# Unalome81/IEEE-802.11-OFDM-QPSK-Simulator

Hardware: AMD Instinct MI355X
Metric: OFDM symbols/sec (whole node) over BER-vs-SNR sweep; achieved HBM GB/s vs peak (higher is better)
Workload: dtype f32

## Files before the change

### ieee-802.11-ofdm-qpsk-simulator_amd/csrc/ofdm_capi.hip

```cpp
#include <hip/hip_runtime.h>
#include <algorithm>
#include <cmath>
#include <cstdint>
#include <cstdlib>
#include <complex>
#include <cstdio>
#include <cstring>
#include <mutex>
#include <string>
#include <vector>
#include "ofdm_internal.h"
#include "ofdm_ctx.h"

using namespace ofdm;

namespace ofdm {

thread_local std::string g_last_error;

int set_error(int code, const char *fmt, ...) {
    char buf[512];
    va_list ap;
    va_start(ap, fmt);
    vsnprintf(buf, sizeof(buf), fmt, ap);
// ... 171 lines not shown
        return set_error(OFDM_E_HIP, "hipStreamCreate failed");
    }
    c->stream = c->own;
    for (int conv = 0; conv < 2; ++conv) {
        std::vector<float2> t;
        host_ltf_time(conv, t);
        std::vector<float2> t2(68 * 2);
        for (int r = 0; r < 68; ++r) {
            const float2 v = t[(r - 4 + 64) & 63];
            t2[2 * r] = t2[2 * r + 1] = make_float2(2.0f * v.x, 2.0f * v.y);
        }
        if (hipMalloc(&c->d_ltf[conv], 64 * sizeof(float2)) != hipSuccess ||
            hipMemcpy(c->d_ltf[conv], t.data(), 64 * sizeof(float2), hipMemcpyHostToDevice) != hipSuccess ||
            hipMalloc(&c->d_ltf2_rows[conv], t2.size() * sizeof(float2)) != hipSuccess ||
            hipMemcpy(c->d_ltf2_rows[conv], t2.data(), t2.size() * sizeof(float2), hipMemcpyHostToDevice) != hipSuccess) {
            ofdm_ctx_destroy(reinterpret_cast<ofdm_ctx *>(c));
            return set_error(OFDM_E_NOMEM, "LTF table upload failed");
        }
    }
    *out = reinterpret_cast<ofdm_ctx *>(c);
    return OFDM_OK;
}

int ofdm_ctx_destroy(ofdm_ctx *ctx) {
    Ctx *c = reinterpret_cast<Ctx *>(ctx);
    if (!c) return OFDM_OK;
    hipSetDevice(c->device);
    hipStreamSynchronize(c->stream);
    for (auto &e : c->done) { hipEventDestroy(e.a); hipEventDestroy(e.b); }
    for (auto &e : c->open) { hipEventDestroy(e.a); hipEventDestroy(e.b); }
    for (auto ev : c->pool) hipEventDestroy(ev);
    if (c->tx_stream) hipStreamSynchronize(c->tx_stream);
    for (void *p : {(void *)c->d_ltf[0], (void *)c->d_ltf[1], (void *)c->d_ltf2_rows[0], (void *)c->d_ltf2_rows[1], c->d_tx, c->d_bits, c->d_cnt, c->d_scratch,
                    c->d_scratch2, c->d_wave, c->d_tx2, c->d_bits2, c->d_work})
        if (p) hipFree(p);
    for (hipEvent_t ev : {c->ev_start, c->ev_tx[0], c->ev_tx[1], c->ev_rx[0], c->ev_rx[1]})
        if (ev) hipEventDestroy(ev);
    if (c->h_cnt) hipHostFree(c->h_cnt);
    if (c->tx_stream) hipStreamDestroy(c->tx_stream);
    if (c->own) hipStreamDestroy(c->own);
    delete c;
    return OFDM_OK;
}

int ofdm_ctx_trim(ofdm_ctx *ctx, int64_t *released) {
    Ctx *c = reinterpret_cast<Ctx *>(ctx);
    if (!c) return set_error(OFDM_E_ARG, "ctx is NULL");
    HIPOK(hipSetDevice(c->device));
    HIPOK(hipStreamSynchronize(c->stream));
    if (c->tx_stream) HIPOK(hipStreamSynchronize(c->tx_stream));
    int64_t n = 0;
    struct { void **p; size_t *cap; } bufs[] = {{&c->d_tx, &c->cap_tx}, {&c->d_bits, &c->cap_bits}, {&c->d_tx2, &c->cap_tx2},
                                                {&c->d_bits2, &c->cap_bits2}, {&c->d_cnt, &c->cap_cnt},
                                                {&c->d_scratch, &c->cap_scratch}, {&c->d_scratch2, &c->cap_scratch2}};
    for (auto &b : bufs) {
        if (*b.p) {
            HIPOK(hipFree(*b.p));
            n += (int64_t)*b.cap;
        }
        *b.p = nullptr;
        *b.cap = 0;
    }
    if (released) *released = n;
    return OFDM_OK;
}

int ofdm_ctx_scratch_bytes(ofdm_ctx *ctx, int64_t *bytes) {
// ... 206 lines not shown
        RxArgs a{};
        a.tx = (const float2 *)d_tx;
        a.bits = (const uint32_t *)d_bits;
        a.ltf = c->d_ltf[cfg->conv];
        a.ltf2_rows = c->d_ltf2_rows[cfg->conv];
        a.first_frame = first_frame;
        a.n_frames = n_frames;
        a.pitch = sym_pitch(n_frames);
        a.k0 = (uint32_t)cfg->seed;
        a.k1 = (uint32_t)(cfg->seed >> 32);
        a.n_snr = std::min(OFDM_MAX_SNR, n_snr - q0);
        a.q_base = q0;
        a.counters = (unsigned long long *)d_counters + (size_t)q0 * OFDM_NCOUNTERS;
        a.dump_frames = n_frames;
        if (dump) {
            a.dump_eq = (float2 *)d_eq + (size_t)q0 * n_frames * 2 * 48;
            a.dump_bits = (uint32_t *)d_dbits + (size_t)q0 * n_frames * 2 * 3;
        }
        for (int q = 0; q < a.n_snr; ++q) {
            const double s2 = cfg->kappa * cfg->p_ref / std::pow(10.0, snr_db[q0 + q] / 10.0);
            a.sigma[q] = (float)std::sqrt(s2);
        }
        if (fuse_nx && q0 == 0) {
            a.nx = tx_args(c, &c->nx_cfg, c->nx_first, c->nx_n, c->nx_tx, c->nx_bits);
            a.nx_conv = c->nx_cfg.conv;
        }
        if (fuse_own && q0 == 0) {
            a.own = tx_args(c, cfg, first_frame, n_frames, const_cast<void *>(d_tx), const_cast<void *>(d_bits));
            a.own_conv = cfg->conv;
        }
        if (!c->d_work) HIPOK(hipMalloc(&c->d_work, 256));
        a.work = (unsigned long long *)c->d_work;
        HIPOK(hipMemsetAsync(c->d_work, 0, sizeof(unsigned long long), c->stream));
        c->tic(Ctx::K_RX);
        launch_rx(c->stream, a, *cfg, dump, grid);
        c->toc();
        HIPOK(hipGetLastError());
    }
    return OFDM_OK;
}

int ofdm_rx_frames(ofdm_ctx *ctx, const ofdm_cfg *cfg, const void *d_tx, const void *d_bits, uint64_t first_frame,
                   int64_t n_frames, const double *snr_db, int n_snr, void *d_counters) {
    return rx_common(reinterpret_cast<Ctx *>(ctx), cfg, d_tx, d_bits, first_frame, n_frames, snr_db, n_snr,
                     d_counters, nullptr, nullptr);
}

int ofdm_rx_frames_dump(ofdm_ctx *ctx, const ofdm_cfg *cfg, const void *d_tx, const void *d_bits,
                        uint64_t first_frame, int64_t n_frames, const double *snr_db, int n_snr, void *d_counters,
                        void *d_eq, void *d_dbits) {
    return rx_common(reinterpret_cast<Ctx *>(ctx), cfg, d_tx, d_bits, first_frame, n_frames, snr_db, n_snr,
                     d_counters, d_eq, d_dbits);
}

int ofdm_txrx_frames(ofdm_ctx *ctx, const ofdm_cfg *cfg, uint64_t first_frame, int64_t n_frames, void *d_tx,
                     void *d_bits, const double *snr_db, int n_snr, void *d_counters) {
    Ctx *c = reinterpret_cast<Ctx *>(ctx);
    int rc = check_tx(c, cfg, n_frames, d_tx, d_bits);
    if (rc) return rc;
    return rx_common(c, cfg, d_tx, d_bits, first_frame, n_frames, snr_db, n_snr, d_counters, nullptr, nullptr, true);
}

int ofdm_symbol_sweep(ofdm_ctx *ctx, const ofdm_cfg *cfg, const double *snr_db, int n_snr, uint64_t first_frame,
                      int64_t n_frames, int64_t chunk_frames, int64_t *counters) {
    Ctx *c = reinterpret_cast<Ctx *>(ctx);
    if (!c) return set_error(OFDM_E_ARG, "ctx is NULL");
// ... 78 lines not shown
```

### ieee-802.11-ofdm-qpsk-simulator_amd/csrc/ofdm_ctx.h

```cpp
#pragma once
#include <hip/hip_runtime.h>
#include <cstdarg>
#include <string>
#include <vector>
#include "ofdm_mi355x_long.h"

namespace ofdm {

int set_error(int code, const char *fmt, ...);
int check_cfg(const ofdm_cfg *c);

constexpr int MSG_MAX_FRAMES = 8;
constexpr int MSG_MAX_CHARS = 12 * MSG_MAX_FRAMES;
int payload_table(int payload, const std::string &message, uint32_t table[3 * MSG_MAX_FRAMES]);
constexpr int LONG_MAX_FRAMES = OFDM_LONG_MAX_DATA_SYMBOLS;
constexpr int LONG_MSG_MAX_CHARS = OFDM_LONG_MSG_MAX_CHARS;
static_assert(LONG_MSG_MAX_CHARS == 12 * LONG_MAX_FRAMES, "12 characters per data symbol");
int payload_table_long(int payload, const std::string &message, uint32_t table[3 * LONG_MAX_FRAMES]);
struct Ctx;
int check_symbol_payload(const Ctx *c, int payload);

struct Ctx {
    enum { K_FFT = 0, K_TX = 1, K_RX = 2, K_FRAME = 3, K_STREAM_DETECT = 4, K_STREAM_SELECT = 5, K_STREAM_DECODE = 6,
           K_TRANSMIT = 7, K_CHANNEL = 8, K_SCORE = 9, K_FADE = 10, K_DRAW_TAPS = 11, K_STREAM_DETECT_CONJ = 12,
           K_STREAM_TIMING = 13, NK = 14 };
    int device = 0;
    int cus = 256;
    hipStream_t own = nullptr;
    hipStream_t stream = nullptr;
    float2 *d_ltf[2] = {nullptr, nullptr};
    float2 *d_ltf2_rows[2] = {nullptr, nullptr};
    std::string message = "Hey! I am Vivaswan";
    void *d_tx = nullptr, *d_bits = nullptr, *d_cnt = nullptr, *d_scratch = nullptr, *d_scratch2 = nullptr;
    void *d_tx2 = nullptr, *d_bits2 = nullptr;
    size_t cap_tx2 = 0, cap_bits2 = 0;
    hipStream_t tx_stream = nullptr;
    bool nx_pending = false;
    ofdm_cfg nx_cfg{};
    uint64_t nx_first = 0;
    int64_t nx_n = 0;
    void *nx_tx = nullptr, *nx_bits = nullptr;
    hipEvent_t ev_start = nullptr, ev_tx[2] = {nullptr, nullptr}, ev_rx[2] = {nullptr, nullptr};
    void *d_wave = nullptr;
    void *d_work = nullptr;
    void *h_cnt = nullptr;
    size_t cap_h_cnt = 0;
    size_t cap_tx = 0, cap_bits = 0, cap_cnt = 0, cap_scratch = 0, cap_scratch2 = 0, cap_wave = 0;
    int wave_key = -1;
    int wave_frames = 0;
    int32_t wave_len = 0;
    double wave_power = 0.0;
    bool ltf_ready[2] = {false, false};
    float2 ltf_template[2][128] = {};
    struct Ev { hipEvent_t a, b; int kernel; };
    bool timing = false;
    std::vector<Ev> open, done;
    std::vector<hipEvent_t> pool;
    double acc_ms[NK] = {};
    int64_t launches[NK] = {};

    void tic(int k);
    void toc();
    void resolve();
    int ensure(void **p, size_t *cap, size_t bytes);
    int read_counters(void *out, size_t bytes);
};

}
```

### ieee-802.11-ofdm-qpsk-simulator_amd/csrc/ofdm_device.h

```cpp
#pragma once
#include <hip/hip_runtime.h>
#include <stdint.h>
#include <type_traits>
#include "twiddle64.h"

namespace ofdm {

template <int B, int E, typename F>
__device__ __forceinline__ void static_for(F &&f) {
    if constexpr (B < E) {
        f(std::integral_constant<int, B>{});
        static_for<B + 1, E>(f);
    }
}

template <typename T>
__device__ __forceinline__ void opaque(T &v) { asm volatile("" : "+v"(v)); }

__device__ __forceinline__ float2 cadd(float2 a, float2 b) { return make_float2(a.x + b.x, a.y + b.y); }
__device__ __forceinline__ float2 csub(float2 a, float2 b) { return make_float2(a.x - b.x, a.y - b.y); }
__device__ __forceinline__ float2 cscale(float2 a, float s) { return make_float2(a.x * s, a.y * s); }
__device__ __forceinline__ float2 cmul(float2 a, float2 b) {
    return make_float2(fmaf(a.x, b.x, -a.y * b.y), fmaf(a.x, b.y, a.y * b.x));
}
// ... 5 lines not shown
constexpr uint32_t PHILOX_W0 = 0x9E3779B9u, PHILOX_W1 = 0xBB67AE85u;
constexpr uint32_t STREAM_BITS = 0xB1750000u;
constexpr uint32_t STREAM_NOISE = 0x5A000000u;
constexpr uint32_t STREAM_CHAN = 0xC4A00000u;
constexpr uint32_t STREAM_START = 0x5B000000u;

__device__ __forceinline__ uint4 philox10(uint32_t c0, uint32_t c1, uint32_t c2, uint32_t c3,
                                          uint32_t k0, uint32_t k1) {
#pragma unroll
    for (int r = 0; r < 10; ++r) {
        const uint64_t p0 = (uint64_t)PHILOX_M0 * c0;
        const uint64_t p1 = (uint64_t)PHILOX_M1 * c2;
        const uint32_t n0 = __builtin_amdgcn_bitop3_b32((uint32_t)(p1 >> 32), c1, k0, 0x96);
        const uint32_t n2 = __builtin_amdgcn_bitop3_b32((uint32_t)(p0 >> 32), c3, k1, 0x96);
        c0 = n0; c1 = (uint32_t)p1; c2 = n2; c3 = (uint32_t)p0;
        k0 += PHILOX_W0; k1 += PHILOX_W1;
    }
    return make_uint4(c0, c1, c2, c3);
}

struct PhiloxHead { uint32_t c1, n2, c3; };
__device__ __forceinline__ PhiloxHead philox_head(uint32_t c0, uint32_t c1, uint32_t c3, uint32_t k1) {
    const uint64_t p0 = (uint64_t)PHILOX_M0 * c0;
    return {c1, (uint32_t)__builtin_amdgcn_bitop3_b32((uint32_t)(p0 >> 32), c3, k1, 0x96), (uint32_t)p0};
}
__device__ __forceinline__ uint4 philox10_c2(const PhiloxHead &h, uint32_t c2, uint32_t k0, uint32_t k1) {
    const uint64_t p1r = (uint64_t)PHILOX_M1 * c2;
    uint32_t c0 = __builtin_amdgcn_bitop3_b32((uint32_t)(p1r >> 32), h.c1, k0, 0x96);
    uint32_t c1 = (uint32_t)p1r, c3 = h.c3;
    c2 = h.n2;
    k0 += PHILOX_W0; k1 += PHILOX_W1;
#pragma unroll
    for (int r = 1; r < 10; ++r) {
        const uint64_t p0 = (uint64_t)PHILOX_M0 * c0;
        const uint64_t p1 = (uint64_t)PHILOX_M1 * c2;
        const uint32_t n0 = __builtin_amdgcn_bitop3_b32((uint32_t)(p1 >> 32), c1, k0, 0x96);
        const uint32_t n2 = __builtin_amdgcn_bitop3_b32((uint32_t)(p0 >> 32), c3, k1, 0x96);
        c0 = n0; c1 = (uint32_t)p1; c2 = n2; c3 = (uint32_t)p0;
        k0 += PHILOX_W0; k1 += PHILOX_W1;
    }
    return make_uint4(c0, c1, c2, c3);
}

struct PhiloxKeysV {
    uint32_t k0[10], k1[10];
    __device__ __forceinline__ void init(uint32_t s0, uint32_t s1) {
#pragma unroll
        for (int r = 0; r < 10; ++r) {
            asm volatile("v_mov_b32 %0, %1" : "=v"(k0[r]) : "s"(s0 + (uint32_t)r * PHILOX_W0));
            asm volatile("v_mov_b32 %0, %1" : "=v"(k1[r]) : "s"(s1 + (uint32_t)r * PHILOX_W1));
        }
    }
};
__device__ __forceinline__ uint4 philox10_c2(const PhiloxHead &h, uint32_t c2, const PhiloxKeysV &k) {
    const uint64_t p1r = (uint64_t)PHILOX_M1 * c2;
    uint32_t c0 = __builtin_amdgcn_bitop3_b32((uint32_t)(p1r >> 32), h.c1, k.k0[0], 0x96);
    uint32_t c1 = (uint32_t)p1r, c3 = h.c3;
    c2 = h.n2;
#pragma unroll
    for (int r = 1; r < 10; ++r) {
        const uint64_t p0 = (uint64_t)PHILOX_M0 * c0;
        const uint64_t p1 = (uint64_t)PHILOX_M1 * c2;
        const uint32_t n0 = __builtin_amdgcn_bitop3_b32((uint32_t)(p1 >> 32), c1, k.k0[r], 0x96);
        const uint32_t n2 = __builtin_amdgcn_bitop3_b32((uint32_t)(p0 >> 32), c3, k.k1[r], 0x96);
        c0 = n0; c1 = (uint32_t)p1; c2 = n2; c3 = (uint32_t)p0;
    }
// ... 261 lines not shown
```

### ieee-802.11-ofdm-qpsk-simulator_amd/csrc/ofdm_internal.h

```cpp
#pragma once
#include <hip/hip_runtime.h>
#include <stdint.h>
#include "ofdm_mi355x.h"
#include "ofdm_device.h"

namespace ofdm {

constexpr int OFDM_MAX_SNR = 64;
constexpr int SYM_SAMPLES = 80;

inline int64_t sym_pitch(int64_t n_frames) { return (2 * n_frames + 63) / 64 * 64 + 64; }
constexpr int TX_BIT_ROWS = 10;
constexpr int64_t MAX_BATCH_FRAMES = int64_t(1) << 23;

constexpr int LS_GROUP_FRAMES = 21;
constexpr int LS_GROUP_SYMS = 42;
constexpr int LS_ROW_F2 = 44;

struct TxArgs {
    float2 *tx;
    uint32_t *bits;
    uint64_t first_symbol;
    int64_t n_sym;
    int64_t pitch;
    uint32_t k0, k1;
    int32_t payload;
    int32_t table_frames;
    uint32_t table[24];
};

struct RxArgs {
    const float2 *tx;
    const uint32_t *bits;
    const float2 *ltf;
    uint64_t first_frame;
    int64_t n_frames;
    int64_t pitch;
    const float2 *ltf2_rows;
    uint32_t k0, k1;
    int32_t n_snr;
    int32_t q_base;
    unsigned long long *counters;
    float2 *dump_eq;
    uint32_t *dump_bits;
    int64_t dump_frames;
    unsigned long long *stamps;
    unsigned long long *work;
    TxArgs nx;
    int32_t nx_conv;
    TxArgs own;
    int32_t own_conv;
    float sigma[OFDM_MAX_SNR];
};

void launch_fft64(hipStream_t st, const float2 *in, float2 *out, int64_t n, int inverse, int conv);
void launch_tx(hipStream_t st, const TxArgs &a, int conv);
void launch_rx(hipStream_t st, const RxArgs &a, const ofdm_cfg &cfg, bool dump, unsigned grid);
int rx_grid(const ofdm_cfg &cfg, int64_t n_frames, int device);
bool rx_pack_applies(const ofdm_cfg &cfg);
void launch_rx_pack(hipStream_t st, const RxArgs &a, const ofdm_cfg &cfg, bool dump, unsigned grid);
int rx_pack_grid(const ofdm_cfg &cfg, int64_t n_frames, int device);
void launch_rx_pack_ideal(hipStream_t st, const RxArgs &a, const ofdm_cfg &cfg, bool dump, unsigned grid);
int rx_pack_ideal_grid(int64_t n_frames, int device);

}
```

### ieee-802.11-ofdm-qpsk-simulator_amd/csrc/ofdm_rxpack.hip

```cpp
#include "ofdm_internal.h"
#include "ofdm_rxcommon.h"

#define OFDM_RX_PACK_WAVES 2
#define OFDM_RX_PACK_IDEAL_WAVES 3

namespace ofdm {

constexpr int PK_FRAMES = 64;
constexpr int PK_SYMS = 2 * PK_FRAMES;

typedef float f4v __attribute__((ext_vector_type(4)));
typedef __attribute__((address_space(3))) const f4v lcf4;
typedef unsigned int u2v __attribute__((ext_vector_type(2)));
typedef __attribute__((address_space(3))) const u2v lcu2;
typedef __attribute__((address_space(3))) f2v lf2;

constexpr int PACK_PF = 2;
constexpr int PACK_GEN_SPLIT = 2;
constexpr int PACK_FENCE_PAIRS = 2;

__host__ __device__ constexpr int rev16(int m) { return ((m & 3) << 2) | (m >> 2); }
__host__ __device__ constexpr int pos32(int k) { return (k & 1) ? 16 + rev16(k >> 1) : rev16(k >> 1); }

template <int K>
// ... 12 lines not shown
        const float2 Hk = chan_bin<k>(h), Hm = chan_bin<64 - k>(h);
        col[p * PK_FRAMES] = make_float4(Hk.x, Hk.y, Hm.x, Hm.y);
        sched_fence();
    });
}

__device__ __forceinline__ void clean_spectrum(const RxArgs &a, int64_t s, float4 *spec_col ) {
    gcf2 *src = (gcf2 *)(a.tx + 16 * a.pitch + s);
    int P = (int)a.pitch;
    opaque(P);
    float2 x[64];
    static_for<0, 4>([&](auto gc) {
        constexpr int g = decltype(gc)::value;
        gcf2 *sp = src;
        opaque(sp);
        static_for<0, 16>([&](auto pc) {
            constexpr int n = 16 * (decltype(pc)::value >> 2) + 4 * g + (decltype(pc)::value & 3);
            const float2 v = gld(sp, n * P);
            x[n] = (n & 1) ? make_float2(-v.x, -v.y) : v;
        });
        static_for<0, 4>([&](auto ic) { dif_stage1<false, 4 * g + decltype(ic)::value>(x); });
        sched_fence();
    });
    auto store = [&](auto pc) {
        constexpr int p = decltype(pc)::value;
        constexpr int k = pair_bin(p);
        const float2 c0 = x[digit_rev4(k)], c1 = x[digit_rev4(64 - k)];
        spec_col[p * 2 * PK_FRAMES] = make_float4(c0.x, c0.y, c1.x, c1.y);
    };
    static_for<0, 4>([&](auto rc) { dif_sub16<false, decltype(rc)::value>(x); });
    static_for<0, PACK_PAIRS>(store);
}

template <int KIND, bool DUMP>
__device__ __forceinline__ void demap_bin(float2 u, float r, uint32_t &t, uint32_t sm, float &evm, uint32_t &em,
                                          int m, float2 *dump_eq, uint32_t (&dbits)[3]) {
    constexpr float cd = KIND == 2 ? 0.5f * INV_SQRT2 : INV_SQRT2;
    const uint32_t ti = t, tr = dbl_u32(t);
    t = dbl_u32(tr);
    const uint32_t ur = __builtin_amdgcn_bitop3_b32(__float_as_uint(u.x), tr, sm, 0x78);
    const uint32_t ui = __builtin_amdgcn_bitop3_b32(__float_as_uint(u.y), ti, sm, 0x78);
    float ex, ey;
    if constexpr (KIND == 0) {
        ex = __uint_as_float(ur) - cd;
        ey = __uint_as_float(ui) - cd;
    } else {
        ex = fmaf(__uint_as_float(ur), r, -cd);
        ey = fmaf(__uint_as_float(ui), r, -cd);
    }
    evm = fmaf(ex, ex, fmaf(ey, ey, evm));
    em = __builtin_amdgcn_alignbit(em, ur, 31);
    em = __builtin_amdgcn_alignbit(em, ui, 31);
    if constexpr (DUMP) {
        const float g = KIND == 0 ? 1.0f : 2.0f * r;
        const float2 z = make_float2(u.x * g, u.y * g);
        if (dump_eq) dump_eq[m] = z;
        const uint32_t pr = z.x > 0.f, pi = z.y > 0.f;
        const int wi = (2 * m) >> 5, s0 = 31 - ((2 * m) & 31), s1 = 31 - ((2 * m + 1) & 31);
        dbits[wi] |= ((pi ^ 1u) << s0) | ((pr ^ pi) << s1);
    }
}

template <typename KS>
__device__ __forceinline__ Noise4 pack_noise(const PhiloxHead &hd, uint32_t c2, const KS &keys, uint32_t k1, float K) {
    uint4 o;
    if constexpr (std::is_same_v<KS, PhiloxKeysV>) o = philox10_c2(hd, c2, keys);
    else o = philox10_c2(hd, c2, keys, k1);
    return noise4_of(o, K);
}

#ifdef OFDM_PACK_STAMPS
#include <cstdio>
static __device__ unsigned long long g_pack_stamps[4][8];
#define PK_STAMP(k)                                                                  \
    do {                                                                             \
        const unsigned long long t_ = __builtin_amdgcn_s_memtime();                  \
        st_acc[k] += t_ - st_t;                                                      \
        st_t = t_;                                                                   \
    } while (0)
#else
#define PK_STAMP(k) do { } while (0)
#endif

#define OFDM_RX_PACK_FADE_WAVES 2
#define PACK_SACC_SUB_LS 4
#define PACK_SACC_SUB 1
template <int KIND, int CONV, int CHAN, bool DUMP>
__global__ __launch_bounds__(256, KIND == 2 ? (CHAN == OFDM_CHAN_RAYLEIGH4 ? OFDM_RX_PACK_FADE_WAVES : OFDM_RX_PACK_WAVES)
                                            : OFDM_RX_PACK_IDEAL_WAVES) void rx_pack_kernel(RxArgs a) {
    constexpr bool FADE = CHAN == OFDM_CHAN_RAYLEIGH4;
    static_assert(!FADE || KIND == 2, "the packed Rayleigh receiver is the LS one");
    constexpr bool WLATE = KIND == 2 && !FADE;
    __shared__ __attribute__((aligned(16))) float4 spec[PACK_PAIRS][2][PK_FRAMES];
    __shared__ __attribute__((aligned(16))) float4 ce[PACK_PAIRS];
    __shared__ __attribute__((aligned(16))) float4 fce[FADE ? PACK_PAIRS : 1][FADE ? PK_FRAMES : 1];
    __shared__ __attribute__((aligned(8))) uint32_t truth[3][PK_SYMS];
    constexpr int SUBN = KIND != 2 ? PACK_SACC_SUB : FADE ? (PACK_SACC_SUB_LS < 4 ? PACK_SACC_SUB_LS : 4)
                                                      : PACK_SACC_SUB_LS;
    constexpr int SACC_XQ = 16;
    __shared__ unsigned long long sacc[OFDM_MAX_SNR][5];
    __shared__ unsigned long long sacx[SUBN > 1 ? SACC_XQ : 1][SUBN > 1 ? 5 * (SUBN - 1) : 1];
    auto slots = [&](int q, int ln) -> unsigned long long * {
        const int c = ln % SUBN;
        return SUBN > 1 && c > 0 && q < SACC_XQ ? &sacx[q][5 * (c - 1)] : sacc[q];
    };
    __shared__ uint32_t pf_dummy[64];
    __shared__ __attribute__((aligned(8))) float2 lds_keep[1];
    const int tid = threadIdx.x, lane = tid & 63;
    const int wv = __builtin_amdgcn_readfirstlane(tid >> 6);
#ifdef OFDM_PACK_STAMPS
    unsigned long long st_acc[8] = {0, 0, 0, 0, 0, 0, 0, 0};
    unsigned long long st_t = __builtin_amdgcn_s_memtime();
#endif
    for (int i = tid; i < a.n_snr * 5; i += blockDim.x) (&sacc[0][0])[i] = 0ull;
    if constexpr (SUBN > 1)
        for (int i = tid; i < SACC_XQ * 5 * (SUBN - 1); i += blockDim.x) (&sacx[0][0])[i] = 0ull;
    if constexpr (KIND == 2) {
        if (wv == 0) {
            float2 x[64];
            static_for<0, 64>([&](auto nc) {
                constexpr int n = decltype(nc)::value;
                const float2 v = a.ltf[n];
                x[n] = (n & 1) ? make_float2(-2.0f * v.x, -2.0f * v.y) : make_float2(2.0f * v.x, 2.0f * v.y);
            });
            fft64<false>(x);
            if (lane == 0) {
                static_for<0, PACK_PAIRS>([&](auto pc) {
                    constexpr int p = decltype(pc)::value;
                    constexpr int k = pair_bin(p);
                    const float2 c0 = x[digit_rev4(k)], c1 = x[digit_rev4(64 - k)];
                    ce[p] = make_float4(c0.x, c0.y, c1.x, c1.y);
                });
            }
        }
    }
    const int64_t n_groups = (a.n_frames + PK_FRAMES - 1) / PK_FRAMES;
    const int B = (int)gridDim.x, G = (int)n_groups, R = G / B, T = G - R * B;
    const int S = T > 0 ? max(1, min(4, B / T)) : 1;
    const int n_items = R * B + T * S;
    __shared__ int next_item;
    for (int w = blockIdx.x; w < n_items; w = __builtin_amdgcn_readfirstlane(next_item)) {
        const bool tail = w >= R * B;
        const int tw = tail ? w - R * B : 0;
        const int64_t grp = tail ? R * B + tw / S : w;
        const int sub = tail ? tw % S : 0, ns = tail ? S : 1;
        __syncthreads();
        PK_STAMP(0);
        int t = tid;
        opaque(t);
        using KArgs = const __attribute__((address_space(4))) RxArgs;
        KArgs *ap = (KArgs *)__builtin_amdgcn_kernarg_segment_ptr();
        asm volatile("" : "+s"(ap));
        const bool own_tx = ap->own.n_sym > 0;
        if (own_tx) {
            if (t >= PK_SYMS) {
                const int64_t sidx = grp * PK_SYMS + (t - PK_SYMS);
                if (sidx < ap->own.n_sym) {
                    if (ap->own_conv == OFDM_CONV_C) tx_symbol<OFDM_CONV_C>(ap->own, sidx);
                    else tx_symbol<OFDM_CONV_MATLAB>(ap->own, sidx);
                }
            }
            __syncthreads();
        }
        if (t < PK_SYMS) {
            clean_spectrum(a, grp * PK_SYMS + t, &spec[0][t & 1][t >> 1]);
        } else {
            const int j = t - PK_SYMS;
            const uint32_t *src = a.bits + 7 * a.pitch + grp * PK_SYMS + j;
            truth[0][j] = src[0];
            truth[1][j] = src[a.pitch];
            truth[2][j] = src[2 * a.pitch];
            if (j < 64) {
                int nx = 0;
                if (j == 0) nx = B + (int)atomicAdd(a.work, 1ull);
                nx = __builtin_amdgcn_readlane(nx, 0);
                if (j == 0) next_item = nx;
                if (nx < n_items && !own_tx && !WLATE) {
                    const int64_t ng = nx < R * B ? nx : R * B + (nx - R * B) / S;
#pragma unroll
                    for (int i = 0; i < 8; ++i) {
                        const int line = j + 64 * i;
                        const float2 *p = a.tx + (int64_t)(16 + (line >> 3)) * a.pitch + ng * PK_SYMS + (line & 7) * 16;
                        __builtin_amdgcn_global_load_lds((__attribute__((address_space(1))) void *)p,
                                                         (__attribute__((address_space(3))) void *)pf_dummy, 4, 0, 0);
                    }
                }
            }
            if (ap->nx.n_sym > 0 && sub == 0) {
                for (int64_t sidx = grp * PK_SYMS + j; sidx < ap->nx.n_sym; sidx += (int64_t)G * PK_SYMS) {
                    if (ap->nx_conv == OFDM_CONV_C) tx_symbol<OFDM_CONV_C>(ap->nx, sidx);
                    else tx_symbol<OFDM_CONV_MATLAB>(ap->nx, sidx);
                }
            }
            if constexpr (FADE) {
                const int fr = j & 63;
                const uint64_t ff = a.first_frame + (uint64_t)(grp * PK_FRAMES + fr);
                float2 h[4];
                channel_taps((uint32_t)ff, (uint32_t)(ff >> 32), a.k0, a.k1, h);
                if (j < 64) chan_pairs<0>(h, &fce[0][fr]);
                else chan_pairs<1>(h, &fce[0][fr]);
            }
        }
        PK_STAMP(1);
        __syncthreads();
        PK_STAMP(2);
        if constexpr (FADE) {
            for (int it = t; it < PACK_PAIRS * PK_FRAMES; it += 256) {
                const int p = it >> 6, fr = it & 63;
                const float4 H = fce[p][fr], c0 = spec[p][0][fr], c1 = spec[p][1][fr], e = ce[p];
                const float2 Hk = make_float2(H.x, H.y), Hm = make_float2(H.z, H.w);
                float2 u = cmul(Hk, make_float2(c0.x, c0.y)), v = cmul(Hm, make_float2(c0.z, c0.w));
                spec[p][0][fr] = make_float4(u.x, u.y, v.x, v.y);
                u = cmul(Hk, make_float2(c1.x, c1.y)); v = cmul(Hm, make_float2(c1.z, c1.w));
                spec[p][1][fr] = make_float4(u.x, u.y, v.x, v.y);
                u = cmul(Hk, make_float2(e.x, e.y)); v = cmul(Hm, make_float2(e.z, e.w));
                fce[p][fr] = make_float4(u.x, u.y, v.x, v.y);
            }
            __syncthreads();
        }
        PK_STAMP(3);
        const int64_t fl = grp * PK_FRAMES + lane;
        const bool valid = fl < a.n_frames;
        const uint64_t f = a.first_frame + (uint64_t)fl;
        for (int q = wv + 4 * sub; q < a.n_snr; q += 4 * ns) {
            if constexpr (WLATE) {
                if (wv == 2 && q + 4 * ns >= a.n_snr) {
                    const int nx = __builtin_amdgcn_readfirstlane(next_item);
                    using KArgsW = const __attribute__((address_space(4))) RxArgs;
                    KArgsW *apw = (KArgsW *)__builtin_amdgcn_kernarg_segment_ptr();
                    if (nx < n_items && apw->own.n_sym == 0) {
                        const int64_t ng = nx < R * B ? nx : R * B + (nx - R * B) / S;
                        const int ln = lane;
#pragma unroll
                        for (int i = 0; i < 8; ++i) {
                            const int line = ln + 64 * i;
                            const float2 *p = a.tx + (int64_t)(16 + (line >> 3)) * a.pitch + ng * PK_SYMS + (line & 7) * 16;
                            __builtin_amdgcn_global_load_lds((__attribute__((address_space(1))) void *)p,
                                                             (__attribute__((address_space(3))) void *)pf_dummy, 4, 0, 0);
                        }
                    }
                }
            }
            uint32_t flo = (uint32_t)f, fhi = (uint32_t)(f >> 32);
            opaque(flo); opaque(fhi);
            const float sigma = a.sigma[q];
            const uint32_t qs = STREAM_NOISE | (uint32_t)(a.q_base + q);
            const PhiloxHead hd = philox_head(flo, fhi, qs, a.k1);
            float2 z[64];
            float2 ee[PACK_PAIRS];
            lf2 *keep = (lf2 *)&lds_keep[0];
            opaque(keep);
            if constexpr (KIND == 2) {
                const float KE = noise_k(sigma * 1.41421356237309504880f);
                static_for<0, 4>([&](auto ic) {
                    constexpr int i = decltype(ic)::value;
                    uint32_t tg = 48u + 2 * i;
                    opaque(tg);
                    static_for<0, 2>([&](auto hc) {
                        constexpr int h = decltype(hc)::value;
                        const Noise4 lo = pack_noise(hd, tg + h, a.k0, a.k1, KE);
                        const Noise4 hi = pack_noise(hd, tg + 8 + h, a.k0, a.k1, KE);
                        constexpr int m = 4 * i + 2 * h;
                        z[m] = make_float2(lo.r0 * lo.c0, -(lo.r0 * lo.s0));
                        z[m + 1] = make_float2(lo.r1 * lo.c1, -(lo.r1 * lo.s1));
                        z[m + 16] = make_float2(hi.r0 * hi.c0, -(hi.r0 * hi.s0));
                        z[m + 17] = make_float2(hi.r1 * hi.c1, -(hi.r1 * hi.s1));
                    });
                    static_for<0, 4>([&](auto jc) {
                        constexpr int j = 4 * i + decltype(jc)::value;
                        const float2 u = z[j], v = z[j + 16];
                        z[j] = cadd(u, v);
                        z[j + 16] = twiddle<2 * j, false>(csub(u, v));
                    });
                    sched_fence();
                });
                dif4<false, 16, 0>(z);
                dif4<false, 16, 16>(z);
                static_for<0, PACK_PAIRS>([&](auto pc) {
                    constexpr int p = decltype(pc)::value;
                    constexpr int k = pair_bin(p);
                    const float2 P = z[pos32(k)], Qv = z[pos32(32 - k)];
                    const float2 F = make_float2(P.x + Qv.x, P.y - Qv.y);
                    const float2 H = twiddle<k, false>(make_float2(P.x - Qv.x, P.y + Qv.y));
                    ee[p] = make_float2(F.x + H.y, F.y - H.x);
                });
                sched_fence();
            }
            const float K = noise_k(sigma);
            float2 x[64];
            static_for<0, 4>([&](auto gc) {
                constexpr int g = decltype(gc)::value;
                uint32_t tg = 84u + g;
                opaque(tg);
                static_for<0, 4>([&](auto Qc) {
                    constexpr int Q = decltype(Qc)::value;
                    const Noise4 n0 = pack_noise(hd, tg + 4 * Q, a.k0, a.k1, K);
                    const Noise4 n1 = pack_noise(hd, tg + 20 + 4 * Q, a.k0, a.k1, K);
                    const float d0[4] = {n0.r0 * n0.c0, n0.r0 * n0.s0, n0.r1 * n0.c1, n0.r1 * n0.s1};
                    const float d1[4] = {n1.r0 * n1.c0, n1.r0 * n1.s0, n1.r1 * n1.c1, n1.r1 * n1.s1};
                    static_for<0, 4>([&](auto ic) {
                        constexpr int i = decltype(ic)::value;
                        x[16 * Q + 4 * g + i] = (i & 1) ? make_float2(-d0[i], -d1[i]) : make_float2(d0[i], d1[i]);
                    });
                    if constexpr (Q % PACK_GEN_SPLIT == PACK_GEN_SPLIT - 1 && Q < 3) sched_fence();
                });
                static_for<0, 4>([&](auto ic) { dif_stage1<false, 4 * g + decltype(ic)::value>(x); });
                sched_fence();
            });
            float2 *deq0 = nullptr, *deq1 = nullptr;
            uint32_t *dbit0 = nullptr, *dbit1 = nullptr;
            if constexpr (DUMP) {
                if (valid) {
                    const int64_t r0 = ((int64_t)q * a.dump_frames + fl) * 2;
                    deq0 = a.dump_eq + r0 * 48; deq1 = deq0 + 48;
                    dbit0 = a.dump_bits + r0 * 3; dbit1 = dbit0 + 3;
                }
            }
            uint32_t db0[3] = {0u, 0u, 0u}, db1[3] = {0u, 0u, 0u};
            lcf4 *sp = (lcf4 *)&spec[0][0][lane];
            lcu2 *tw = (lcu2 *)&truth[0][2 * lane];
            lcf4 *fp = (lcf4 *)&fce[0][FADE ? lane : 0];
            opaque(sp); opaque(tw);
            if constexpr (FADE) opaque(fp);
            uint32_t sm;
            asm volatile("v_mov_b32 %0, 0x80000000" : "=v"(sm));
            float evm = 0.f;
            uint32_t em = 0u, be = 0u, ax = 0u, t0 = 0u, t1 = 0u;
            constexpr int PF = KIND == 2 && !FADE ? PACK_PF : 0;
            f4v pc0[PF + 1], pc1[PF + 1];
            float4 pe4[PF + 1];
            auto load_pair = [&](auto pc) {
                constexpr int p = decltype(pc)::value;
                if constexpr (p < PACK_PAIRS) {
                    constexpr int slot = p % (PF + 1);
                    pc0[slot] = sp[p * 2 * PK_FRAMES];
                    pc1[slot] = sp[(p * 2 + 1) * PK_FRAMES];
                    if constexpr (KIND == 2) {
                        if constexpr (FADE) {
                            const f4v v = fp[p * PK_FRAMES];
                            pe4[slot] = make_float4(v.x, v.y, v.z, v.w);
                        } else {
                            pe4[slot] = ce[p];
                        }
                    }
                }
            };
            if constexpr (PF > 0) static_for<0, PF>(load_pair);
            auto pair = [&](auto pc) {
                constexpr int p = decltype(pc)::value;
                constexpr int k = pair_bin(p), k2 = 64 - k;
                if constexpr ((p & 7) == 0) {
                    const u2v tt = tw[(p >> 3) * (PK_SYMS / 2)];
                    t0 = tt.x; t1 = tt.y;
                }
                if constexpr (PF > 0) load_pair(std::integral_constant<int, p + PF>{});
                constexpr int slot = p % (PF + 1);
                const float2 Zk = x[digit_rev4(k)], Zm = x[digit_rev4(k2)];
                const float2 A = make_float2(Zk.x + Zm.x, Zk.y - Zm.y), B = make_float2(Zk.x - Zm.x, Zk.y + Zm.y);
                if constexpr (PF == 0) load_pair(pc);
                const f4v c0 = pc0[slot], c1 = pc1[slot];
                const float2 y0k = make_float2(fmaf(0.5f, A.x, c0.x), fmaf(0.5f, A.y, c0.y));
                const float2 y0m = make_float2(fmaf(0.5f, A.x, c0.z), fmaf(-0.5f, A.y, c0.w));
                const float2 y1k = make_float2(fmaf(0.5f, B.y, c1.x), fmaf(-0.5f, B.x, c1.y));
                const float2 y1m = make_float2(fmaf(0.5f, B.y, c1.z), fmaf(0.5f, B.x, c1.w));
                float2 u0k, u0m, u1k, u1m;
                float rk = 0.f, rm = 0.f;
                if constexpr (KIND == 2) {
                    const float ex = ee[p].x, ey = ee[p].y;
                    const float4 e4 = pe4[slot];
                    const float2 Sk = make_float2(fmaf(0.5f, ex, e4.x), fmaf(0.5f, ey, e4.y));
                    const float2 Sm = make_float2(fmaf(0.5f, ex, e4.z), fmaf(-0.5f, ey, e4.w));
                    rk = __builtin_amdgcn_rcpf(fmaf(Sk.x, Sk.x, Sk.y * Sk.y));
                    rm = __builtin_amdgcn_rcpf(fmaf(Sm.x, Sm.x, Sm.y * Sm.y));
                    u0k = cscale(cmulc(y0k, Sk), (float)ltf_sign(k));
                    u1k = cscale(cmulc(y1k, Sk), (float)ltf_sign(k));
                    u0m = cscale(cmulc(y0m, Sm), (float)ltf_sign(k2));
                    u1m = cscale(cmulc(y1m, Sm), (float)ltf_sign(k2));
                } else {
                    constexpr float cs = (CONV == OFDM_CONV_C && (k & 1)) ? -1.0f : 1.0f;
                    u0k = cscale(y0k, cs); u0m = cscale(y0m, cs); u1k = cscale(y1k, cs); u1m = cscale(y1m, cs);
                }
                demap_bin<KIND, DUMP>(u0k, rk, t0, sm, evm, em, data_index(k), deq0, db0);
                demap_bin<KIND, DUMP>(u0m, rm, t0, sm, evm, em, data_index(k2), deq0, db0);
                demap_bin<KIND, DUMP>(u1k, rk, t1, sm, evm, em, data_index(k), deq1, db1);
                demap_bin<KIND, DUMP>(u1m, rm, t1, sm, evm, em, data_index(k2), deq1, db1);
                if constexpr ((p & 3) == 3) {
                    ax += __popc(em);
                    be += __popc(em & 0x55555555u) + __popc((em ^ (em >> 1)) & 0x55555555u);
                    em = 0u;
                }
                opaque(evm);
                if constexpr (p % PACK_FENCE_PAIRS == PACK_FENCE_PAIRS - 1) sched_fence();
            };
            dif_sub16<false, 0>(x);
            static_for<0, 6>(pair);
            sched_fence();
            dif_sub16<false, 2>(x);
            static_for<6, 13>(pair);
            sched_fence();
            dif_sub16<false, 1>(x);
            dif_sub16<false, 3>(x);
            static_for<13, 24>(pair);
            if constexpr (DUMP) {
                if (dbit0) {
                    dbit0[0] = db0[0]; dbit0[1] = db0[1]; dbit0[2] = db0[2];
                    dbit1[0] = db1[0]; dbit1[1] = db1[1]; dbit1[2] = db1[2];
                }
            }
            FrameAcc acc;
            frame_metrics(acc, KIND == 2 ? 4.0f * evm : evm, be, ax);
            flush_lanes(acc, valid, slots(q, lane));
        }
        PK_STAMP(4);
    }
    if constexpr (SUBN > 1) {
        __syncthreads();
        for (int i = tid; i < min(a.n_snr, SACC_XQ) * 5; i += 256) {
            const int q = i / 5, k = i % 5;
            unsigned long long v = sacc[q][k];
#pragma unroll
            for (int c = 1; c < SUBN; ++c) v += sacx[q][5 * (c - 1) + k];
            sacc[q][k] = v;
        }
    }
    block_flush(a, sacc, tid);
    PK_STAMP(5);
#ifdef OFDM_PACK_STAMPS
    if (lane == 0)
        for (int k = 0; k < 6; ++k) atomicAdd(&g_pack_stamps[wv][k], st_acc[k]);
#endif
}

template <int KIND, int CONV, int CHAN = OFDM_CHAN_AWGN>
static void launch_pack_t(hipStream_t st, const RxArgs &a, bool dump, unsigned grid) {
    if (dump) hipLaunchKernelGGL((rx_pack_kernel<KIND, CONV, CHAN, true>), dim3(grid), dim3(256), 0, st, a);
    else hipLaunchKernelGGL((rx_pack_kernel<KIND, CONV, CHAN, false>), dim3(grid), dim3(256), 0, st, a);
#ifdef OFDM_PACK_STAMPS
    unsigned long long hs[4][8];
    if (hipStreamSynchronize(st) == hipSuccess && hipMemcpyFromSymbol(hs, HIP_SYMBOL(g_pack_stamps), sizeof hs) == hipSuccess) {
        static const char *names[6] = {"item-top barrier", "prologue work", "prologue barrier", "faded spectra",
                                       "SNR loop", "block flush"};
        for (int w : {0, 2}) {
            double tot = 0;
            for (int k = 0; k < 6; ++k) tot += (double)hs[w][k];
            fprintf(stderr, "pack stamp wave %d:", w);
// ... 1 lines not shown
            fprintf(stderr, "\n");
        }
    }
#endif
}

template <const void *(*K)()>
static int pack_grid(int64_t n_frames, int device) {
    const int64_t need = (n_frames + PK_FRAMES - 1) / PK_FRAMES;
    int per_cu = 0, cus = 0;
    if (hipOccupancyMaxActiveBlocksPerMultiprocessor(&per_cu, K(), 256, 0) != hipSuccess || per_cu < 1) per_cu = 1;
    if (hipDeviceGetAttribute(&cus, hipDeviceAttributeMultiprocessorCount, device) != hipSuccess || cus < 1) cus = 256;
    const int64_t cap = (int64_t)per_cu * cus;
    const int64_t g = need < cap ? need : cap;
    return (int)(g < 1 ? 1 : g);
}

#ifdef OFDM_RXPACK_IDEAL_TU
static const void *ideal_kernel() { return reinterpret_cast<const void *>(&rx_pack_kernel<0, OFDM_CONV_C, OFDM_CHAN_AWGN, false>); }

void launch_rx_pack_ideal(hipStream_t st, const RxArgs &a, const ofdm_cfg &cfg, bool dump, unsigned grid) {
    if (cfg.conv == OFDM_CONV_C) launch_pack_t<0, OFDM_CONV_C>(st, a, dump, grid);
    else launch_pack_t<0, OFDM_CONV_MATLAB>(st, a, dump, grid);
}

int rx_pack_ideal_grid(int64_t n_frames, int device) { return pack_grid<ideal_kernel>(n_frames, device); }
#else
bool rx_pack_applies(const ofdm_cfg &cfg) {
    if (cfg.noise != OFDM_NOISE_REAL) return false;
    if (cfg.channel == OFDM_CHAN_RAYLEIGH4) return cfg.est == OFDM_EST_LS;
    return cfg.channel == OFDM_CHAN_AWGN;
}

void launch_rx_pack(hipStream_t st, const RxArgs &a, const ofdm_cfg &cfg, bool dump, unsigned grid) {
    if (cfg.est == OFDM_EST_LS && cfg.channel == OFDM_CHAN_RAYLEIGH4)
        launch_pack_t<2, OFDM_CONV_C, OFDM_CHAN_RAYLEIGH4>(st, a, dump, grid);
    else if (cfg.est == OFDM_EST_LS) launch_pack_t<2, OFDM_CONV_C>(st, a, dump, grid);
    else launch_rx_pack_ideal(st, a, cfg, dump, grid);
}

static const void *ls_kernel() { return reinterpret_cast<const void *>(&rx_pack_kernel<2, OFDM_CONV_C, OFDM_CHAN_AWGN, false>); }
static const void *fade_kernel() {
    return reinterpret_cast<const void *>(&rx_pack_kernel<2, OFDM_CONV_C, OFDM_CHAN_RAYLEIGH4, false>);
}

int rx_pack_grid(const ofdm_cfg &cfg, int64_t n_frames, int device) {
    if (cfg.est != OFDM_EST_LS) return rx_pack_ideal_grid(n_frames, device);
    return cfg.channel == OFDM_CHAN_RAYLEIGH4 ? pack_grid<fade_kernel>(n_frames, device)
                                              : pack_grid<ls_kernel>(n_frames, device);
}
#endif

}
```

Before: 12.59 billion.

## Precompute frame-invariant Philox words on host and read truth bits from constellation

Splits the Philox noise generator so that the parts depending only on the high frame word and block index are precomputed once per key on the host. They are uploaded as a small table, staged into LDS per group, and the first rounds are then skipped on device. For non-fading channels it also drops the per-symbol truth-bit loads and derives the demap sign from the known constellation with bitop3. A fast and a slow SNR loop are both instantiated, chosen by whether a frame group shares its high word. This adds code size, LDS use and host-side table maintenance with stream syncs when the key changes.

```diff
diff --git a/ieee-802.11-ofdm-qpsk-simulator_amd/csrc/ofdm_capi.hip b/ieee-802.11-ofdm-qpsk-simulator_amd/csrc/ofdm_capi.hip
--- a/ieee-802.11-ofdm-qpsk-simulator_amd/csrc/ofdm_capi.hip
+++ b/ieee-802.11-ofdm-qpsk-simulator_amd/csrc/ofdm_capi.hip
@@ -227,7 +227,7 @@
     for (auto ev : c->pool) hipEventDestroy(ev);
     if (c->tx_stream) hipStreamSynchronize(c->tx_stream);
     for (void *p : {(void *)c->d_ltf[0], (void *)c->d_ltf[1], (void *)c->d_ltf2_rows[0], (void *)c->d_ltf2_rows[1], c->d_tx, c->d_bits, c->d_cnt, c->d_scratch,
-                    c->d_scratch2, c->d_wave, c->d_tx2, c->d_bits2, c->d_work})
+                    c->d_scratch2, c->d_wave, c->d_tx2, c->d_bits2, c->d_work, c->d_philox})
         if (p) hipFree(p);
     for (hipEvent_t ev : {c->ev_start, c->ev_tx[0], c->ev_tx[1], c->ev_rx[0], c->ev_rx[1]})
         if (ev) hipEventDestroy(ev);
@@ -500,6 +500,21 @@
         if (!c->d_work) HIPOK(hipMalloc(&c->d_work, 256));
         a.work = (unsigned long long *)c->d_work;
         HIPOK(hipMemsetAsync(c->d_work, 0, sizeof(unsigned long long), c->stream));
+        if (rx_pack_applies(*cfg)) {
+            static_assert(sizeof(c->h_philox) == sizeof(PhiloxWords[2][PACK_BLOCKS]), "table size");
+            const uint32_t key[3] = {a.k0, a.k1, (uint32_t)(first_frame >> 32)};
+            if (!c->d_philox) HIPOK(hipMalloc(&c->d_philox, sizeof(c->h_philox)));
+            if (!c->philox_valid || c->philox_stream != c->stream || std::memcmp(key, c->philox_key, sizeof key)) {
+                if (c->philox_valid) HIPOK(hipStreamSynchronize(c->philox_stream));
+                c->philox_valid = false;
+                pack_philox_table(key[0], key[1], key[2], *reinterpret_cast<PhiloxWords (*)[2][PACK_BLOCKS]>(c->h_philox));
+                HIPOK(hipMemcpyAsync(c->d_philox, c->h_philox, sizeof(c->h_philox), hipMemcpyHostToDevice, c->stream));
+                std::memcpy(c->philox_key, key, sizeof key);
+                c->philox_stream = c->stream;
+                c->philox_valid = true;
+            }
+            a.philox_words = (const PhiloxWords *)c->d_philox;
+        }
         c->tic(Ctx::K_RX);
         launch_rx(c->stream, a, *cfg, dump, grid);
         c->toc();
diff --git a/ieee-802.11-ofdm-qpsk-simulator_amd/csrc/ofdm_ctx.h b/ieee-802.11-ofdm-qpsk-simulator_amd/csrc/ofdm_ctx.h
--- a/ieee-802.11-ofdm-qpsk-simulator_amd/csrc/ofdm_ctx.h
+++ b/ieee-802.11-ofdm-qpsk-simulator_amd/csrc/ofdm_ctx.h
@@ -43,6 +43,11 @@
     hipEvent_t ev_start = nullptr, ev_tx[2] = {nullptr, nullptr}, ev_rx[2] = {nullptr, nullptr};
     void *d_wave = nullptr;
     void *d_work = nullptr;
+    void *d_philox = nullptr;
+    bool philox_valid = false;
+    uint32_t philox_key[3] = {0, 0, 0};
+    hipStream_t philox_stream = nullptr;
+    uint32_t h_philox[2 * 48 * 4] = {};
     void *h_cnt = nullptr;
     size_t cap_h_cnt = 0;
     size_t cap_tx = 0, cap_bits = 0, cap_cnt = 0, cap_scratch = 0, cap_scratch2 = 0, cap_wave = 0;
diff --git a/ieee-802.11-ofdm-qpsk-simulator_amd/csrc/ofdm_device.h b/ieee-802.11-ofdm-qpsk-simulator_amd/csrc/ofdm_device.h
--- a/ieee-802.11-ofdm-qpsk-simulator_amd/csrc/ofdm_device.h
+++ b/ieee-802.11-ofdm-qpsk-simulator_amd/csrc/ofdm_device.h
@@ -61,6 +61,42 @@
     k0 += PHILOX_W0; k1 += PHILOX_W1;
 #pragma unroll
     for (int r = 1; r < 10; ++r) {
+        const uint64_t p0 = (uint64_t)PHILOX_M0 * c0;
+        const uint64_t p1 = (uint64_t)PHILOX_M1 * c2;
+        const uint32_t n0 = __builtin_amdgcn_bitop3_b32((uint32_t)(p1 >> 32), c1, k0, 0x96);
+        const uint32_t n2 = __builtin_amdgcn_bitop3_b32((uint32_t)(p0 >> 32), c3, k1, 0x96);
+        c0 = n0; c1 = (uint32_t)p1; c2 = n2; c3 = (uint32_t)p0;
+        k0 += PHILOX_W0; k1 += PHILOX_W1;
+    }
+    return make_uint4(c0, c1, c2, c3);
+}
+
+struct PhiloxWords { uint32_t x, y, z, pad; };
+__host__ __device__ inline PhiloxWords philox_words(uint32_t c1, uint32_t c2, uint32_t k0, uint32_t k1) {
+    const uint64_t p1 = (uint64_t)PHILOX_M1 * c2;
+    const uint32_t c0n = (uint32_t)(p1 >> 32) ^ c1 ^ k0;
+    const uint64_t p0 = (uint64_t)PHILOX_M0 * c0n;
+    return {(uint32_t)p1 ^ (k0 + PHILOX_W0), (uint32_t)(p0 >> 32) ^ (k1 + PHILOX_W1),
+            (uint32_t)p0 ^ (k1 + 2u * PHILOX_W1), 0u};
+}
+struct PhiloxMid { uint32_t p1lo, p1hi, c3; };
+__device__ __forceinline__ PhiloxMid philox_mid(const PhiloxHead &h) {
+    const uint64_t p1 = (uint64_t)PHILOX_M1 * h.n2;
+    return {(uint32_t)p1, (uint32_t)(p1 >> 32), h.c3};
+}
+__device__ __forceinline__ uint4 philox10_c2(const PhiloxMid &m, uint32_t wx, uint32_t wy, uint32_t wz, uint32_t k0,
+                                             uint32_t k1) {
+    uint32_t c0 = m.p1hi ^ wx, c1 = m.p1lo, c2 = m.c3 ^ wy, c3;
+    k0 += 2u * PHILOX_W0; k1 += 2u * PHILOX_W1;
+    {
+        const uint64_t p0 = (uint64_t)PHILOX_M0 * c0;
+        const uint64_t p1 = (uint64_t)PHILOX_M1 * c2;
+        const uint32_t n0 = __builtin_amdgcn_bitop3_b32((uint32_t)(p1 >> 32), c1, k0, 0x96);
+        c0 = n0; c1 = (uint32_t)p1; c2 = (uint32_t)(p0 >> 32) ^ wz; c3 = (uint32_t)p0;
+        k0 += PHILOX_W0; k1 += PHILOX_W1;
+    }
+#pragma unroll
+    for (int r = 3; r < 10; ++r) {
         const uint64_t p0 = (uint64_t)PHILOX_M0 * c0;
         const uint64_t p1 = (uint64_t)PHILOX_M1 * c2;
         const uint32_t n0 = __builtin_amdgcn_bitop3_b32((uint32_t)(p1 >> 32), c1, k0, 0x96);
diff --git a/ieee-802.11-ofdm-qpsk-simulator_amd/csrc/ofdm_internal.h b/ieee-802.11-ofdm-qpsk-simulator_amd/csrc/ofdm_internal.h
--- a/ieee-802.11-ofdm-qpsk-simulator_amd/csrc/ofdm_internal.h
+++ b/ieee-802.11-ofdm-qpsk-simulator_amd/csrc/ofdm_internal.h
@@ -46,12 +46,17 @@
     int64_t dump_frames;
     unsigned long long *stamps;
     unsigned long long *work;
+    const PhiloxWords *philox_words;
     TxArgs nx;
     int32_t nx_conv;
     TxArgs own;
     int32_t own_conv;
     float sigma[OFDM_MAX_SNR];
 };
+
+constexpr int PACK_BLOCKS = 48;
+constexpr uint32_t pack_block(int slot) { return slot < 16 ? 48u + slot : slot < 32 ? 84u + (slot - 16) : 104u + (slot - 32); }
+void pack_philox_table(uint32_t k0, uint32_t k1, uint32_t frame_hi, PhiloxWords (&out)[2][PACK_BLOCKS]);
 
 void launch_fft64(hipStream_t st, const float2 *in, float2 *out, int64_t n, int inverse, int conv);
 void launch_tx(hipStream_t st, const TxArgs &a, int conv);
diff --git a/ieee-802.11-ofdm-qpsk-simulator_amd/csrc/ofdm_rxpack.hip b/ieee-802.11-ofdm-qpsk-simulator_amd/csrc/ofdm_rxpack.hip
--- a/ieee-802.11-ofdm-qpsk-simulator_amd/csrc/ofdm_rxpack.hip
+++ b/ieee-802.11-ofdm-qpsk-simulator_amd/csrc/ofdm_rxpack.hip
@@ -68,14 +68,20 @@
     static_for<0, PACK_PAIRS>(store);
 }
 
-template <int KIND, bool DUMP>
-__device__ __forceinline__ void demap_bin(float2 u, float r, uint32_t &t, uint32_t sm, float &evm, uint32_t &em,
-                                          int m, float2 *dump_eq, uint32_t (&dbits)[3]) {
+template <int KIND, bool DUMP, bool WALK, int TBL>
+__device__ __forceinline__ void demap_bin(float2 u, float r, uint32_t &t, float sx, float sy, uint32_t sm, float &evm,
+                                          uint32_t &em, int m, float2 *dump_eq, uint32_t (&dbits)[3]) {
     constexpr float cd = KIND == 2 ? 0.5f * INV_SQRT2 : INV_SQRT2;
-    const uint32_t ti = t, tr = dbl_u32(t);
-    t = dbl_u32(tr);
-    const uint32_t ur = __builtin_amdgcn_bitop3_b32(__float_as_uint(u.x), tr, sm, 0x78);
-    const uint32_t ui = __builtin_amdgcn_bitop3_b32(__float_as_uint(u.y), ti, sm, 0x78);
+    uint32_t ur, ui;
+    if constexpr (WALK) {
+        const uint32_t ti = t, tr = dbl_u32(t);
+        t = dbl_u32(tr);
+        ur = __builtin_amdgcn_bitop3_b32(__float_as_uint(u.x), tr, sm, 0x78);
+        ui = __builtin_amdgcn_bitop3_b32(__float_as_uint(u.y), ti, sm, 0x78);
+    } else {
+        ur = __builtin_amdgcn_bitop3_b32(__float_as_uint(u.x), __float_as_uint(sx), sm, TBL);
+        ui = __builtin_amdgcn_bitop3_b32(__float_as_uint(u.y), __float_as_uint(sy), sm, TBL);
+    }
     float ex, ey;
     if constexpr (KIND == 0) {
         ex = __uint_as_float(ur) - cd;
@@ -103,6 +109,14 @@
     if constexpr (std::is_same_v<KS, PhiloxKeysV>) o = philox10_c2(hd, c2, keys);
     else o = philox10_c2(hd, c2, keys, k1);
     return noise4_of(o, K);
+}
+
+typedef unsigned int u4v __attribute__((ext_vector_type(4)));
+static_assert(sizeof(PhiloxWords) == sizeof(u4v), "one 16-byte read per block");
+typedef __attribute__((address_space(3))) const u4v cwords;
+__device__ __forceinline__ Noise4 pack_noise(const PhiloxMid &md, cwords *w, uint32_t k0, uint32_t k1, float K) {
+    const u4v v = *w;
+    return noise4_of(philox10_c2(md, v.x, v.y, v.z, k0, k1), K);
 }
 
 #ifdef OFDM_PACK_STAMPS
@@ -130,7 +144,7 @@
     __shared__ __attribute__((aligned(16))) float4 spec[PACK_PAIRS][2][PK_FRAMES];
     __shared__ __attribute__((aligned(16))) float4 ce[PACK_PAIRS];
     __shared__ __attribute__((aligned(16))) float4 fce[FADE ? PACK_PAIRS : 1][FADE ? PK_FRAMES : 1];
-    __shared__ __attribute__((aligned(8))) uint32_t truth[3][PK_SYMS];
+    __shared__ __attribute__((aligned(8))) uint32_t truth[FADE ? 3 : 1][FADE ? PK_SYMS : 2];
     constexpr int SUBN = KIND != 2 ? PACK_SACC_SUB : FADE ? (PACK_SACC_SUB_LS < 4 ? PACK_SACC_SUB_LS : 4)
                                                       : PACK_SACC_SUB_LS;
     constexpr int SACC_XQ = 16;
@@ -140,6 +154,7 @@
         const int c = ln % SUBN;
         return SUBN > 1 && c > 0 && q < SACC_XQ ? &sacx[q][5 * (c - 1)] : sacc[q];
     };
+    __shared__ __attribute__((aligned(16))) u4v wlds[PACK_BLOCKS];
     __shared__ uint32_t pf_dummy[64];
     __shared__ __attribute__((aligned(8))) float2 lds_keep[1];
     const int tid = threadIdx.x, lane = tid & 63;
@@ -182,6 +197,9 @@
         const int sub = tail ? tw % S : 0, ns = tail ? S : 1;
         __syncthreads();
         PK_STAMP(0);
+        const uint64_t fg = a.first_frame + (uint64_t)(grp * PK_FRAMES);
+        const uint32_t row = (uint32_t)(fg >> 32) - (uint32_t)(a.first_frame >> 32);
+        const bool uniform_hi = (uint32_t)((fg + (PK_FRAMES - 1)) >> 32) == (uint32_t)(fg >> 32) && row < 2u;
         int t = tid;
         opaque(t);
         using KArgs = const __attribute__((address_space(4))) RxArgs;
@@ -202,10 +220,12 @@
             clean_spectrum(a, grp * PK_SYMS + t, &spec[0][t & 1][t >> 1]);
         } else {
             const int j = t - PK_SYMS;
-            const uint32_t *src = a.bits + 7 * a.pitch + grp * PK_SYMS + j;
-            truth[0][j] = src[0];
-            truth[1][j] = src[a.pitch];
-            truth[2][j] = src[2 * a.pitch];
+            if constexpr (FADE) {
+                const uint32_t *src = a.bits + 7 * a.pitch + grp * PK_SYMS + j;
+                truth[0][j] = src[0];
+                truth[1][j] = src[a.pitch];
+                truth[2][j] = src[2 * a.pitch];
+            }
             if (j < 64) {
                 int nx = 0;
                 if (j == 0) nx = B + (int)atomicAdd(a.work, 1ull);
@@ -228,6 +248,8 @@
                     else tx_symbol<OFDM_CONV_MATLAB>(ap->nx, sidx);
                 }
             }
+            if (uniform_hi && j >= 64 && j < 64 + PACK_BLOCKS)
+                wlds[j - 64] = ((const u4v *)a.philox_words)[row * PACK_BLOCKS + (j - 64)];
             if constexpr (FADE) {
                 const int fr = j & 63;
                 const uint64_t ff = a.first_frame + (uint64_t)(grp * PK_FRAMES + fr);
@@ -258,6 +280,9 @@
         const int64_t fl = grp * PK_FRAMES + lane;
         const bool valid = fl < a.n_frames;
         const uint64_t f = a.first_frame + (uint64_t)fl;
+        auto snr_loop = [&](auto fastc) __attribute__((always_inline)) {
+        constexpr bool FAST = decltype(fastc)::value;
+        cwords *wtab = (cwords *)&wlds[0];
         for (int q = wv + 4 * sub; q < a.n_snr; q += 4 * ns) {
             if constexpr (WLATE) {
                 if (wv == 2 && q + 4 * ns >= a.n_snr) {
@@ -282,6 +307,12 @@
             const float sigma = a.sigma[q];
             const uint32_t qs = STREAM_NOISE | (uint32_t)(a.q_base + q);
             const PhiloxHead hd = philox_head(flo, fhi, qs, a.k1);
+            const PhiloxMid md = philox_mid(hd);
+            cwords *wt = wtab;
+            auto noise = [&](uint32_t blk, int slot, float Kn) __attribute__((always_inline)) {
+                if constexpr (FAST) return pack_noise(md, wt + slot, a.k0, a.k1, Kn);
+                else return pack_noise(hd, blk, a.k0, a.k1, Kn);
+            };
             float2 z[64];
             float2 ee[PACK_PAIRS];
             lf2 *keep = (lf2 *)&lds_keep[0];
@@ -291,11 +322,12 @@
                 static_for<0, 4>([&](auto ic) {
                     constexpr int i = decltype(ic)::value;
                     uint32_t tg = 48u + 2 * i;
-                    opaque(tg);
+                    if constexpr (FAST) opaque(wt);
+                    else opaque(tg);
                     static_for<0, 2>([&](auto hc) {
                         constexpr int h = decltype(hc)::value;
-                        const Noise4 lo = pack_noise(hd, tg + h, a.k0, a.k1, KE);
-                        const Noise4 hi = pack_noise(hd, tg + 8 + h, a.k0, a.k1, KE);
+                        const Noise4 lo = noise(tg + h, 2 * i + h, KE);
+                        const Noise4 hi = noise(tg + 8 + h, 2 * i + 8 + h, KE);
                         constexpr int m = 4 * i + 2 * h;
                         z[m] = make_float2(lo.r0 * lo.c0, -(lo.r0 * lo.s0));
                         z[m + 1] = make_float2(lo.r1 * lo.c1, -(lo.r1 * lo.s1));
@@ -327,11 +359,12 @@
             static_for<0, 4>([&](auto gc) {
                 constexpr int g = decltype(gc)::value;
                 uint32_t tg = 84u + g;
-                opaque(tg);
+                if constexpr (FAST) opaque(wt);
+                else opaque(tg);
                 static_for<0, 4>([&](auto Qc) {
                     constexpr int Q = decltype(Qc)::value;
-                    const Noise4 n0 = pack_noise(hd, tg + 4 * Q, a.k0, a.k1, K);
-                    const Noise4 n1 = pack_noise(hd, tg + 20 + 4 * Q, a.k0, a.k1, K);
+                    const Noise4 n0 = noise(tg + 4 * Q, 16 + g + 4 * Q, K);
+                    const Noise4 n1 = noise(tg + 20 + 4 * Q, 32 + g + 4 * Q, K);
                     const float d0[4] = {n0.r0 * n0.c0, n0.r0 * n0.s0, n0.r1 * n0.c1, n0.r1 * n0.s1};
                     const float d1[4] = {n1.r0 * n1.c0, n1.r0 * n1.s0, n1.r1 * n1.c1, n1.r1 * n1.s1};
                     static_for<0, 4>([&](auto ic) {
@@ -354,9 +387,10 @@
             }
             uint32_t db0[3] = {0u, 0u, 0u}, db1[3] = {0u, 0u, 0u};
             lcf4 *sp = (lcf4 *)&spec[0][0][lane];
-            lcu2 *tw = (lcu2 *)&truth[0][2 * lane];
+            lcu2 *tw = (lcu2 *)&truth[0][FADE ? 2 * lane : 0];
             lcf4 *fp = (lcf4 *)&fce[0][FADE ? lane : 0];
-            opaque(sp); opaque(tw);
+            opaque(sp);
+            if constexpr (FADE) opaque(tw);
             if constexpr (FADE) opaque(fp);
             uint32_t sm;
             asm volatile("v_mov_b32 %0, 0x80000000" : "=v"(sm));
@@ -385,7 +419,7 @@
             auto pair = [&](auto pc) {
                 constexpr int p = decltype(pc)::value;
                 constexpr int k = pair_bin(p), k2 = 64 - k;
-                if constexpr ((p & 7) == 0) {
+                if constexpr (FADE && (p & 7) == 0) {
                     const u2v tt = tw[(p >> 3) * (PK_SYMS / 2)];
                     t0 = tt.x; t1 = tt.y;
                 }
@@ -416,10 +450,11 @@
                     constexpr float cs = (CONV == OFDM_CONV_C && (k & 1)) ? -1.0f : 1.0f;
                     u0k = cscale(y0k, cs); u0m = cscale(y0m, cs); u1k = cscale(y1k, cs); u1m = cscale(y1m, cs);
                 }
-                demap_bin<KIND, DUMP>(u0k, rk, t0, sm, evm, em, data_index(k), deq0, db0);
-                demap_bin<KIND, DUMP>(u0m, rm, t0, sm, evm, em, data_index(k2), deq0, db0);
-                demap_bin<KIND, DUMP>(u1k, rk, t1, sm, evm, em, data_index(k), deq1, db1);
-                demap_bin<KIND, DUMP>(u1m, rm, t1, sm, evm, em, data_index(k2), deq1, db1);
+                constexpr int TBL = (CONV == OFDM_CONV_C && (k & 1)) ? 0xD2 : 0x78;
+                demap_bin<KIND, DUMP, FADE, TBL>(u0k, rk, t0, c0.x, c0.y, sm, evm, em, data_index(k), deq0, db0);
+                demap_bin<KIND, DUMP, FADE, TBL>(u0m, rm, t0, c0.z, c0.w, sm, evm, em, data_index(k2), deq0, db0);
+                demap_bin<KIND, DUMP, FADE, TBL>(u1k, rk, t1, c1.x, c1.y, sm, evm, em, data_index(k), deq1, db1);
+                demap_bin<KIND, DUMP, FADE, TBL>(u1m, rm, t1, c1.z, c1.w, sm, evm, em, data_index(k2), deq1, db1);
                 if constexpr ((p & 3) == 3) {
                     ax += __popc(em);
                     be += __popc(em & 0x55555555u) + __popc((em ^ (em >> 1)) & 0x55555555u);
@@ -447,6 +482,9 @@
             frame_metrics(acc, KIND == 2 ? 4.0f * evm : evm, be, ax);
             flush_lanes(acc, valid, slots(q, lane));
         }
+        };
+        if (uniform_hi) snr_loop(std::true_type{});
+        else snr_loop(std::false_type{});
         PK_STAMP(4);
     }
     if constexpr (SUBN > 1) {
@@ -514,10 +552,18 @@
     return cfg.channel == OFDM_CHAN_AWGN;
 }
 
+void pack_philox_table(uint32_t k0, uint32_t k1, uint32_t frame_hi, PhiloxWords (&out)[2][PACK_BLOCKS]) {
+    for (int r = 0; r < 2; ++r)
+        for (int s = 0; s < PACK_BLOCKS; ++s) out[r][s] = philox_words(frame_hi + (uint32_t)r, pack_block(s), k0, k1);
+}
+
 void launch_rx_pack(hipStream_t st, const RxArgs &a, const ofdm_cfg &cfg, bool dump, unsigned grid) {
     if (cfg.est == OFDM_EST_LS && cfg.channel == OFDM_CHAN_RAYLEIGH4)
         launch_pack_t<2, OFDM_CONV_C, OFDM_CHAN_RAYLEIGH4>(st, a, dump, grid);
-    else if (cfg.est == OFDM_EST_LS) launch_pack_t<2, OFDM_CONV_C>(st, a, dump, grid);
+    else if (cfg.est == OFDM_EST_LS) {
+        if (cfg.conv == OFDM_CONV_C) launch_pack_t<2, OFDM_CONV_C>(st, a, dump, grid);
+        else launch_pack_t<2, OFDM_CONV_MATLAB>(st, a, dump, grid);
+    }
     else launch_rx_pack_ideal(st, a, cfg, dump, grid);
 }
 
```

After: 13.00 billion, median of 6. +3.3%, better.
